# hjxwhy/mipnerf_pl

Measured on NVIDIA H100. Metric: rays/sec (4096-ray batch, 128+128 samples), higher is better.
Workload: dtype bf16

## Files before the change

mipnerf_pl_b200/csrc/mlp_tc.cu:

```cuda
#include "mlp_tc.h"

#include <algorithm>
#include <cstdlib>
#include <mutex>

#include "kernels.h"
#include "profile.h"
#include "ray_math.cuh"
#include "ray_resample.cuh"
#include "tc_common.cuh"

namespace mipnerf {
namespace {

using namespace tc;

constexpr int kN = 128;
constexpr int kWidth = 256;
constexpr int kCond = 128;
constexpr int kFeat = 96;
constexpr int kViewDim = 27;
constexpr int kNumLayers = 10;
constexpr uint32_t kStageBytes = 16384;
constexpr uint32_t kTailBytes = 8192;
// ... 169 lines not shown

template <int kFmt>
__device__ __forceinline__ float2 unpack2(uint32_t v) {
  if (kFmt == 1) return __bfloat1622float2(*reinterpret_cast<__nv_bfloat162*>(&v));
  return __half22float2(*reinterpret_cast<__half2*>(&v));
}
template <int kFmt>
__device__ __forceinline__ void store8_split(uint8_t* dst_hi, uint8_t* dst_lo, const float (&x)[8]) {
  uint32_t h[4], l[4];
#pragma unroll
  for (int e = 0; e < 4; ++e) {
    h[e] = pack2<kFmt>(x[2 * e], x[2 * e + 1]);
    const float2 f = unpack2<kFmt>(h[e]);
    l[e] = pack2<kFmt>(x[2 * e] - f.x, x[2 * e + 1] - f.y);
  }
  *reinterpret_cast<uint4*>(dst_hi) = make_uint4(h[0], h[1], h[2], h[3]);
  *reinterpret_cast<uint4*>(dst_lo) = make_uint4(l[0], l[1], l[2], l[3]);
}

template <int kFmt, bool kX3, int kT, bool kDensity = false>
__device__ __forceinline__ void ipe_row_group(const LevelParams& p, const RayGeom& g, int64_t ray, int row, float t0,
                                              float t1, uint8_t* myF, int gi_begin, int gi_end) {
  float mean[3] = {0.f, 0.f, 0.f}, cov[3] = {0.f, 0.f, 0.f};
  const float* fin = nullptr;
  if (kDensity) {
    const int64_t pt = ray * kN + row;
    if (pt < p.num_points) {
#pragma unroll
      for (int c = 0; c < 3; ++c) {
        mean[c] = __ldg(p.q_means + pt * 3 + c);
        cov[c] = p.q_covs && !p.disable_integration ? __ldg(p.q_covs + pt * 3 + c) : 0.f;
      }
    }
  } else if (kT == 1 && p.feat_in) {
    fin = p.feat_in + (ray * kN + row) * kFeat;
  } else {
    float tm, tv, rv;
    frustum_moments(t0, t1, g.radius_sq, tm, tv, rv);
    lift_gaussian(g, tm, tv, rv, mean, cov);
    if (p.disable_integration) cov[0] = cov[1] = cov[2] = 0.f;
  }
#pragma unroll
  for (int gi = 0; gi < 6; ++gi) {
    if (gi < gi_begin || gi >= gi_end) continue;
    float fsin[8], fcos[8];
    if (fin) {
#pragma unroll
      for (int e = 0; e < 8; ++e) {
        fsin[e] = __ldg(fin + gi * 8 + e);
        fcos[e] = __ldg(fin + 48 + gi * 8 + e);
      }
    } else {
#pragma unroll
      for (int e = 0; e < 8; ++e) {
        const int f = gi * 8 + e;
        ipe_pair<!kDensity>(mean[f % 3], cov[f % 3], f / 3, fsin[e], fcos[e]);
      }
    }
    const uint32_t o_sin = sw128_offset(row, gi * 8);
    const uint32_t o_cos = gi < 2 ? sw128_offset(row, 48 + gi * 8)
                                  : kStageBytes + sw64_offset(row, (gi - 2) * 8);
    if (kX3) {
      store8_split<kFmt>(myF + o_sin, myF + kFBytes + o_sin, fsin);
      store8_split<kFmt>(myF + o_cos, myF + kFBytes + o_cos, fcos);
    } else {
      store8<kFmt>(myF + o_sin, fsin);
      store8<kFmt>(myF + o_cos, fcos);
    }
  }
}

constexpr int kThreads = 384;
constexpr int kHelperWarp0 = 9;
constexpr int kHelperThreads = 96;
constexpr int kHelperBar = 3;
constexpr int kHeadsWriters = 2 * 128 / 4;
#ifndef MIPNERF_LEVEL_PRODUCER_REGS
#define MIPNERF_LEVEL_PRODUCER_REGS 40
#endif
constexpr int kProducerRegs = MIPNERF_LEVEL_PRODUCER_REGS;
constexpr int kConsumerRegs = (65536 / 128 - kProducerRegs) / 2 / 8 * 8;
static_assert(2 * 128 * kConsumerRegs + 128 * kProducerRegs <= 65536 && kProducerRegs % 8 == 0, "setmaxnreg split");
#ifndef MIPNERF_LEVEL_STAGES
#define MIPNERF_LEVEL_STAGES 6
#endif
template <bool kX3, int kT>
struct LevelLayout {
  static constexpr int kFeatBufs = kX3 ? 1 : 2;
  static constexpr uint32_t kFBuf = (kX3 ? 2 : 1) * kFBytes;
  static constexpr int kStages = kX3 ? 2 : MIPNERF_LEVEL_STAGES;
  static constexpr uint32_t kStage = 16384;
  static constexpr uint32_t kA = 0;
  static constexpr uint32_t kF = kA + (kX3 ? 2 * kABytes : 0);
  static constexpr uint32_t kW = kF + kFeatBufs * kFBuf;
  static constexpr uint32_t kMisc = kW + kStages * kStage;
  static constexpr int kNumMbars = 2 * kStages + 2 * kFeatBufs + 2 * 2;
  static constexpr uint32_t kMiscBytes =
      kNumMbars * 8 + 2 * kN * 4 * 4 + 4 * kT * 4 + 4 * kT * 8 * 4 + (kT * kN + 1) * 4;
  static constexpr uint32_t kVBias = (kMisc + kMiscBytes + 15) & ~15u;
  static constexpr uint32_t kVBiasBytes = 2 * kCond * 4;
  static constexpr uint32_t kPhase = kVBias + kVBiasBytes;
  static constexpr uint32_t kTotal = kPhase + kPhaseBytes + 1024;
  static_assert(kT == 1 || kT == 2, "a ray is one or two 128-row tiles");
  static_assert(kNumMbars % 2 == 0, "the raw heads behind the mbarriers must be 16-B aligned");
  static_assert(kTotal <= 232448, "exceeds 227 KB of shared memory per CTA");
  static_assert(kX3 || kStages * kStage > 72 * 1024 || kTotal + 1024 <= 132 * 1024,
                "bf16 / fp16 with a weight ring of up to 72 KB no longer fits the 132 KB carveout");
  static_assert(kX3 || kStages * kStage > 96 * 1024 || kTotal + 1024 <= 164 * 1024,
                "bf16 / fp16 with a weight ring of up to 96 KB no longer fits the 164 KB carveout");
  static_assert(kX3 ? kStage == 2 * w_stage(false, 0, 0).bytes : kStage == w_stage(true, 1, 0).bytes,
                "a ring slot holds one stage (split modes: its hi and lo stages)");
};

__device__ __forceinline__ bool level_reads_feat(int l, int k) { return l == 0 || (l == 5 && k >= kWidth); }
__device__ __forceinline__ uint64_t level_a_desc(int l, int k, uint32_t a_u, uint32_t f_u, uint32_t ft_u) {
  if (!level_reads_feat(l, k)) return make_sw128_desc(a_u + (uint32_t)(k >> 6) * kStageBytes + 2u * (uint32_t)(k & 63));
  const int kf = l == 0 ? k : k - kWidth;
  if (kf < 64) return make_sw128_desc(f_u + 2u * (uint32_t)kf);
  return make_sw64_desc(ft_u + 2u * (uint32_t)(kf - 64));
}

struct RingPos {
  int st;
  uint32_t ph;
  int prev;
};

template <bool kX3>
__device__ __forceinline__ uint32_t level_stage_acquire(uint32_t w_u, uint64_t* w_full, const RingPos& rp,
                                                        PhaseClock& clk) {
  mbar_wait(&w_full[rp.st], rp.ph);
  clk.mark(kPhWFull);
  wgmma_fence();
  return w_u + (uint32_t)rp.st * LevelLayout<kX3, 1>::kStage;
}
template <bool kX3>
__device__ __forceinline__ void level_stage_commit(uint64_t* w_empty, RingPos& rp, bool leader, PhaseClock& clk) {
  wgmma_commit();
  wgmma_wait<1>();
  if (rp.prev >= 0 && leader) mbar_arrive(&w_empty[rp.prev]);
  rp.prev = rp.st;
  if (++rp.st == LevelLayout<kX3, 1>::kStages) {
    rp.st = 0;
    rp.ph ^= 1;
  }
  clk.mark(kPhMma);
}
template <int kFmt, bool kX3>
__device__ __forceinline__ void level_mma_slab(float (&acc)[64], int l, int s, uint32_t a_u, uint32_t f_u,
                                               uint32_t ft_u, uint32_t w_u, uint64_t* w_full, uint64_t* w_empty,
                                               RingPos& rp, bool leader, PhaseClock& clk) {
  const uint32_t b_u = level_stage_acquire<kX3>(w_u, w_full, rp, clk);
  const WStage ws = w_stage(!kX3, l, s);
#pragma unroll
  for (int j = 0; j < 4; ++j) {
    if (16 * j >= ws.kw) break;
    const uint64_t a_hi = level_a_desc(l, ws.k0 + 16 * j, a_u, f_u, ft_u);
    const uint64_t b_hi = ws.sw128 ? make_sw128_desc(b_u + 32u * j) : make_sw64_desc(b_u + 32u * j);
    wgmma_m64n128k16<kFmt>(acc, a_hi, b_hi, (s | j) ? 1u : 0u);
    if (kX3) {
      wgmma_m64n128k16<kFmt>(acc, a_hi + (level_reads_feat(l, ws.k0) ? kFBytes : kABytes) / 16, b_hi, 1u);
      wgmma_m64n128k16<kFmt>(acc, a_hi, b_hi + ws.bytes / 16, 1u);
    }
  }
  level_stage_commit<kX3>(w_empty, rp, leader, clk);
}
template <int kFmt>
__device__ __forceinline__ void level_mma_slab_rs(float (&acc)[64], const uint32_t (&x)[64], int s, uint32_t w_u,
                                                  uint64_t* w_full, uint64_t* w_empty, RingPos& rp, bool leader,
                                                  PhaseClock& clk) {
  const uint32_t b_u = level_stage_acquire<false>(w_u, w_full, rp, clk);
#pragma unroll
  for (int j = 0; j < 4; ++j) {
    const uint32_t a[4] = {x[16 * s + 4 * j], x[16 * s + 4 * j + 1], x[16 * s + 4 * j + 2], x[16 * s + 4 * j + 3]};
    wgmma_m64n128k16_rs<kFmt>(acc, a, make_sw128_desc(b_u + 32u * j), (s | j) ? 1u : 0u);
  }
  level_stage_commit<false>(w_empty, rp, leader, clk);
}

constexpr int kEpiChunks = 4;
constexpr int kEpiGroups = 16 / kEpiChunks;
constexpr int kEpiOverlap = 1;
static_assert(kEpiOverlap >= 1 && kEpiOverlap + kEpiChunks <= 8, "chunk c must follow the retirement of K-slab c");

struct EpiConsts {
  float2 b[kEpiGroups];
};
__device__ __forceinline__ void level_epilogue_consts(EpiConsts& e, int l, int c_base, int chunk, int cq,
                                                      const SmallParams* __restrict__ gsp) {
#pragma unroll
  for (int jj = 0; jj < kEpiGroups; ++jj)
    e.b[jj] = __ldg(reinterpret_cast<const float2*>(gsp->bias[l] + c_base + 8 * (kEpiGroups * chunk + jj) + cq));
}

template <int kFmt, bool kX3>
__device__ __forceinline__ void level_epilogue_chunk(const float (&acc)[64], const EpiConsts& e, int l, int c_base,
                                                     int chunk, int r0, int cq, uint8_t* sA,
                                                     const SmallParams* __restrict__ gsp, float& d0, float& d1) {
  const bool relu = l < 8;
  uint32_t row_off = (uint32_t)r0 * 128u + 2u * (uint32_t)cq, sw = (uint32_t)(r0 & 7) << 4;
  asm volatile("" : "+r"(row_off), "+r"(sw));
#pragma unroll
  for (int jj = 0; jj < kEpiGroups; ++jj) {
    const int j = kEpiGroups * chunk + jj;
    const float2 b = e.b[jj];
    float a0 = acc[4 * j], a1 = acc[4 * j + 1], a2 = acc[4 * j + 2], a3 = acc[4 * j + 3];
    fadd2(a0, a1, b.x, b.y);
    fadd2(a2, a3, b.x, b.y);
    if (l == 7) {
      const float2 wd = __ldg(reinterpret_cast<const float2*>(gsp->w_density + c_base + 8 * j + cq));
      ffma2(d0, d1, fmaxf(a0, 0.f), fmaxf(a2, 0.f), wd.x, wd.x);
      ffma2(d0, d1, fmaxf(a1, 0.f), fmaxf(a3, 0.f), wd.y, wd.y);
    }
    if (relu) a0 = fmaxf(a0, 0.f), a1 = fmaxf(a1, 0.f), a2 = fmaxf(a2, 0.f), a3 = fmaxf(a3, 0.f);
    const uint32_t o0 = (uint32_t)((c_base >> 6) + (j >> 3)) * kStageBytes + (row_off | ((uint32_t)(j & 7) << 4 ^ sw));
    const uint32_t o1 = o0 + 8u * 128u;
    const uint32_t h0 = pack2<kFmt>(a0, a1), h1 = pack2<kFmt>(a2, a3);
    *reinterpret_cast<uint32_t*>(sA + o0) = h0;
    *reinterpret_cast<uint32_t*>(sA + o1) = h1;
    if (kX3) {
      const float2 f0 = unpack2<kFmt>(h0), f1 = unpack2<kFmt>(h1);
      *reinterpret_cast<uint32_t*>(sA + kABytes + o0) = pack2<kFmt>(a0 - f0.x, a1 - f0.y);
      *reinterpret_cast<uint32_t*>(sA + kABytes + o1) = pack2<kFmt>(a2 - f1.x, a3 - f1.y);
    }
  }
}

#ifndef MIPNERF_LEVEL_EPI_FIRST
#define MIPNERF_LEVEL_EPI_FIRST 4
#endif
constexpr int kEpiFirstRs = MIPNERF_LEVEL_EPI_FIRST;
static_assert(kEpiFirstRs >= 0 && kEpiFirstRs + kEpiChunks <= 8, "the chunks must follow K-slabs 0..3");
__host__ __device__ constexpr int epi_slab_acc0(int c) { return (kEpiFirstRs + c) / 2; }
__host__ __device__ constexpr int epi_slab_acc1(int c) { return c / 2; }
static_assert(epi_slab_acc1(kEpiChunks - 1) < 2, "acc1's chunks must land before the next layer's K-slab 2 reads them");

struct LevelRsCtx {
  uint32_t f_u, ft_u, w_u;
  uint64_t* w_full;
  uint64_t* w_empty;
  uint64_t* feat_empty;
  const SmallParams* gsp;
  uint8_t* dump;
  size_t dump_stride;
  uint64_t dump_policy;
  int r0, cq;
  bool leader;
};

template <int kFmt>
__device__ __forceinline__ void level_epilogue_chunk_rs(const float (&acc)[64], const EpiConsts& e, int l, int c_base,
                                                        int chunk, uint32_t (&x)[64], const LevelRsCtx& k, float& d0,
                                                        float& d1) {
  const bool relu = l < 8;
  uint8_t* dump = k.dump ? k.dump + (size_t)l * k.dump_stride : nullptr;
#pragma unroll
  for (int jj = 0; jj < kEpiGroups; ++jj) {
    const int j = kEpiGroups * chunk + jj;
    const float2 b = e.b[jj];
    float a0 = acc[4 * j], a1 = acc[4 * j + 1], a2 = acc[4 * j + 2], a3 = acc[4 * j + 3];
    fadd2(a0, a1, b.x, b.y);
    fadd2(a2, a3, b.x, b.y);
    if (l == 7) {
      const float2 wd = __ldg(reinterpret_cast<const float2*>(k.gsp->w_density + c_base + 8 * j + k.cq));
      ffma2(d0, d1, fmaxf(a0, 0.f), fmaxf(a2, 0.f), wd.x, wd.x);
      ffma2(d0, d1, fmaxf(a1, 0.f), fmaxf(a3, 0.f), wd.y, wd.y);
    }
    if (relu) a0 = fmaxf(a0, 0.f), a1 = fmaxf(a1, 0.f), a2 = fmaxf(a2, 0.f), a3 = fmaxf(a3, 0.f);
    const int jg = (c_base >> 3) + j;
    x[2 * jg] = pack2<kFmt>(a0, a1);
    x[2 * jg + 1] = pack2<kFmt>(a2, a3);
  }
  if (dump) {
    const int q = k.cq >> 1;
    const int jg = (c_base >> 3) + kEpiGroups * chunk + q;
    const uint32_t o0 = (uint32_t)(jg >> 3) * kStageBytes + sw128_offset(k.r0, 8 * (jg & 7));
#pragma unroll
    for (int h = 0; h < 2; ++h) {
      uint32_t v[4];
#pragma unroll
      for (int jj = 0; jj < 4; ++jj) v[jj] = x[2 * ((c_base >> 3) + kEpiGroups * chunk + jj) + h];
#pragma unroll
      for (int i = 0; i < 2; ++i) {
        const uint32_t r = __shfl_xor_sync(0xffffffffu, (q & 2) ? v[i] : v[2 + i], 2);
        if (q & 2) v[i] = r;
        else v[2 + i] = r;
      }
#pragma unroll
      for (int i = 0; i < 2; ++i) {
        const uint32_t r = __shfl_xor_sync(0xffffffffu, (q & 1) ? v[2 * i] : v[2 * i + 1], 1);
        if (q & 1) v[2 * i] = r;
        else v[2 * i + 1] = r;
      }
      st_global_v4_hint(dump + o0 + (uint32_t)h * 8u * 128u, make_uint4(v[0], v[1], v[2], v[3]), k.dump_policy);
    }
  }
}

template <int kFmt>
__device__ __forceinline__ void level_rs_next_head(float (&acc0)[64], float (&acc1)[64], uint32_t (&x)[64], int l,
                                                   bool release_feat, const LevelRsCtx& k, RingPos& rp, PhaseClock& clk,
                                                   float& d0, float& d1) {
  wgmma_fence_acc(acc0);
#pragma unroll
  for (int s = 0; s < 2; ++s) {
    EpiConsts e[kEpiChunks];
#pragma unroll
    for (int c = 0; c < kEpiChunks; ++c)
      if (epi_slab_acc1(c) == s) level_epilogue_consts(e[c], l, 128, c, k.cq, k.gsp);
    level_mma_slab_rs<kFmt>(acc0, x, s, k.w_u, k.w_full, k.w_empty, rp, k.leader, clk);
    if (s == 0 && release_feat && k.leader) mbar_arrive(k.feat_empty);
    if (s == 0) wgmma_fence_acc(acc1);
#pragma unroll
    for (int c = 0; c < kEpiChunks; ++c)
      if (epi_slab_acc1(c) == s) level_epilogue_chunk_rs<kFmt>(acc1, e[c], l, 128, c, x, k, d0, d1);
    clk.mark(kPhEpilogue);
  }
}

template <int kFmt, bool kSkip, bool kLast = false>
__device__ __forceinline__ void level_rs_layer(float (&acc0)[64], float (&acc1)[64], const uint32_t (&x_in)[64],
                                               uint32_t (&x_out)[64], int l, const LevelRsCtx& k, RingPos& rp,
                                               PhaseClock& clk, float& d0, float& d1) {
  const bool skip = kSkip && l == 5;
  uint32_t f_u = k.f_u, ft_u = k.ft_u;
  asm volatile("" : "+r"(f_u), "+r"(ft_u));
#pragma unroll
  for (int s = 2; s < kWidth / 64; ++s)
    level_mma_slab_rs<kFmt>(acc0, x_in, s, k.w_u, k.w_full, k.w_empty, rp, k.leader, clk);
  if (skip) {
#pragma unroll
    for (int s = kWidth / 64; s < num_slabs(true, 5); ++s)
      level_mma_slab<kFmt, false>(acc0, 5, s, 0u, f_u, ft_u, k.w_u, k.w_full, k.w_empty, rp, k.leader, clk);
  }
  wgmma_fence_acc(acc1);
#pragma unroll
  for (int s = 0; s < kWidth / 64; ++s) {
    EpiConsts e[kEpiChunks];
#pragma unroll
    for (int c = 0; c < kEpiChunks; ++c)
      if (epi_slab_acc0(c) == s) level_epilogue_consts(e[c], l, 0, c, k.cq, k.gsp);
    level_mma_slab_rs<kFmt>(acc1, x_in, s, k.w_u, k.w_full, k.w_empty, rp, k.leader, clk);
    if (s == epi_slab_acc0(0)) wgmma_fence_acc(acc0);
#pragma unroll
    for (int c = 0; c < kEpiChunks; ++c)
      if (epi_slab_acc0(c) == s) level_epilogue_chunk_rs<kFmt>(acc0, e[c], l, 0, c, x_out, k, d0, d1);
    clk.mark(kPhEpilogue);
  }
  if (skip) {
#pragma unroll
    for (int s = kWidth / 64; s < num_slabs(true, 5); ++s)
      level_mma_slab<kFmt, false>(acc1, 5, s, 0u, f_u, ft_u, k.w_u, k.w_full, k.w_empty, rp, k.leader, clk);
  }
  if constexpr (kLast) {
    wgmma_wait<0>();
    wgmma_fence_acc(acc1);
    if (k.leader) mbar_arrive(&k.w_empty[rp.prev]);
    rp.prev = -1;
    clk.mark(kPhMma);
#pragma unroll
    for (int c = 0; c < kEpiChunks; ++c) {
      EpiConsts e;
      level_epilogue_consts(e, l, 128, c, k.cq, k.gsp);
      level_epilogue_chunk_rs<kFmt>(acc1, e, l, 128, c, x_out, k, d0, d1);
    }
    clk.mark(kPhEpilogue);
  } else {
    level_rs_next_head<kFmt>(acc0, acc1, x_out, l, skip, k, rp, clk, d0, d1);
  }
}

__device__ __forceinline__ float quad_sum(float v) {
  v += __shfl_xor_sync(0xffffffffu, v, 1);
  return v + __shfl_xor_sync(0xffffffffu, v, 2);
}

constexpr int kViewPts = 4;
__device__ __forceinline__ float view_enc_elem(const float* vd, int f, int num_deg) {
  float enc;
  if (f < 3) {
    enc = __ldg(vd + f);
  } else {
    const int gidx = f - 3, half = 3 * num_deg, is_cos = gidx >= half, h = is_cos ? gidx - half : gidx;
    const float y = __fmul_rn(__ldg(vd + h % 3), __int_as_float((127 + h / 3) << 23));
    enc = sinf(is_cos ? __fadd_rn(y, MIPNERF_HALF_PI_F32) : y);
  }
  return enc;
}
__device__ __forceinline__ void level_view_terms(const LevelParams& p, int64_t tile, float* slot, int hw, int lane) {
  const float4* wt = reinterpret_cast<const float4*>(p.wimage + kViewDirOffset);
  const float4 b4 = __ldg(wt + kViewDim * kCond / 4 + lane);
#pragma unroll 1
  for (int r = kViewPts * hw; r < kN; r += kViewPts * (kHelperThreads / 32)) {
    float enc[kViewPts];
#pragma unroll
    for (int q = 0; q < kViewPts; ++q) {
      const int64_t pt = tile * kN + r + q;
      enc[q] = 0.f;
      if (lane < kViewDim && pt < p.num_points) {
        const float* vd = p.viewdirs + pt * 3;
        if (lane < 3) {
          enc[q] = __ldg(vd + lane);
        } else {
          const int gidx = lane - 3, is_cos = gidx >= 12, h = is_cos ? gidx - 12 : gidx;
          const float y = __fmul_rn(__ldg(vd + h % 3), __int_as_float((127 + h / 3) << 23));
          enc[q] = sinf(is_cos ? __fadd_rn(y, MIPNERF_HALF_PI_F32) : y);
        }
      }
    }
    float acc[kViewPts][4];
#pragma unroll
    for (int q = 0; q < kViewPts; ++q) acc[q][0] = b4.x, acc[q][1] = b4.y, acc[q][2] = b4.z, acc[q][3] = b4.w;
#pragma unroll 3
    for (int k = 0; k < kViewDim; ++k) {
      const float4 w4 = __ldg(wt + k * (kCond / 4) + lane);
#pragma unroll
      for (int q = 0; q < kViewPts; ++q) {
        const float e = __shfl_sync(0xffffffffu, enc[q], k);
        acc[q][0] = fmaf(w4.x, e, acc[q][0]);
        acc[q][1] = fmaf(w4.y, e, acc[q][1]);
        acc[q][2] = fmaf(w4.z, e, acc[q][2]);
        acc[q][3] = fmaf(w4.w, e, acc[q][3]);
      }
    }
#pragma unroll
    for (int q = 0; q < kViewPts; ++q)
      __stcg(reinterpret_cast<float4*>(slot + (r + q) * kCond) + lane,
             make_float4(acc[q][0], acc[q][1], acc[q][2], acc[q][3]));
  }
  __threadfence_block();
}

template <int kFmt, bool kX3, int kT, int kMode = kModeForward>
__device__ __forceinline__ void level_prepare_tile(const LevelParams& p, int64_t ray, int tt, uint8_t* fbuf,
                                                   float* rs_scratch, int ht, int hw, int lane, PhaseClock& clk,
                                                   float* vb_slot, float* vslot = nullptr) {
  constexpr int kNs = kT * kN;
  constexpr bool kDensity = kMode != kModeForward;
  if constexpr (kMode == kModeRadiance) {
    level_view_terms(p, ray, vslot, hw, lane);
    clk.mark(kPhPrologue);
  }
  if (!kDensity && (kT == 1 || tt == 0)) {
    if (hw == 0) {
      float* t_ray = p.t + ray * (kNs + 1);
      if (p.t_mode == 1) {
        const float nr = __ldg(p.near + ray), fr = __ldg(p.far + ray);
        const bool jit = draws_active(p.t_rand);
// ... 254 lines not shown
            mbar_wait(&feat_empty[fb], ((uint32_t)(j / Lay::kFeatBufs) & 1u) ^ 1u);
            clk.mark(kPhFeatEmpty);
            level_prepare_tile<kFmt, kX3, kT, kMode>(
                p, ray, tt, sF + fb * Lay::kFBuf, rs_scratch, ht, hw, lane, clk, vbias + (i & 1) * kCond,
                kMode == kModeRadiance ? p.view_bias + ((size_t)blockIdx.x * 2 + (j & 1)) * (kN * kCond) : nullptr);
            mbar_arrive(&feat_full[fb]);
          }
          if (tt == 0 && i > 0) {
            const int par = (int)(((i - 1) * kT) & 1);
#pragma unroll
            for (int u = 0; u < kT; ++u)
              mbar_wait(&heads_full[par + u], (uint32_t)(((i - 1) * kT + u) >> 1) & 1u);
            clk.mark(kPhHeadsFull);
            if constexpr (kDensity || kMode == kModeViewAcc)
              level_density_out(p, ray - gridDim.x, heads + par * kN * 4, &heads_empty[par], ht, clk);
            else if constexpr (kMode == kModeRadiance)
              level_radiance_out(p, ray - gridDim.x, heads + par * kN * 4, &heads_empty[par], ht, clk);
            else
              level_composite_ray<kT>(p, ray - gridDim.x, heads + par * kN * 4, &heads_empty[par], cs, ps, ht, hw, lane,
                                      clk);
          }
        }
        if (!more) break;
      }
      clk.end(phase_slot, 3);
      return;
    }
    if (lane == 0) {
      clk.begin(phase_rows + 2 * kNumPhases, true);
      int st = 0;
      uint32_t ph = 0;
      const uint64_t pol = l2_policy_evict_last();
      for (int64_t tile = 0, ray = blockIdx.x; ray < p.num_rays; ray += ++tile % kT == 0 ? gridDim.x : 0) {
        const uint8_t* src = p.wimage;
        for (int l = 0; l < (kDensity ? 8 : kNumLayers); ++l)
          for (int h = 0; h < num_halves(l); ++h)
            for (int s = 0; s < num_slabs(!kX3, l); ++s) {
              const uint32_t bytes = w_stage(!kX3, l, s).bytes;
              clk.mark(kPhIssue);
              mbar_wait(&w_empty[st], ph ^ 1);
              clk.mark(kPhWEmpty);
              mbar_arrive_expect_tx(&w_full[st], kX3 ? 2 * bytes : bytes);
              bulk_g2s_hint(sW + st * Lay::kStage, src, bytes, &w_full[st], pol);
              if (kX3) bulk_g2s_hint(sW + st * Lay::kStage + bytes, src + kLoOffset, bytes, &w_full[st], pol);
              src += bytes;
              if (++st == Lay::kStages) {
                st = 0;
                ph ^= 1;
              }
            }
      }
      clk.mark(kPhIssue);
      clk.end(phase_slot, 2);
    }
    return;
  }

  asm volatile("setmaxnreg.inc.sync.aligned.u32 %0;\n" ::"n"(kConsumerRegs) : "memory");
  const int wg = warp >> 2, t = tid & 127, wq = warp & 3;
  const int r0 = 64 * wg + 16 * wq + (lane >> 2);
  const int cq = 2 * (lane & 3);
  const bool leader = t == 0;
  const SmallParams* __restrict__ gsp = reinterpret_cast<const SmallParams*>(p.wimage + kSmallOffset);
  const uint32_t a_u = smem_u32(sA) + (uint32_t)wg * 64u * 128u;
  const uint32_t w_u = smem_u32(sW);
  const uint64_t dump_policy =
      (kMode != kModeRadiance || kQueryDump) && kT == 1 && p.act_dump ? l2_policy_evict_first() : 0ull;
  bool dump_pending = false;
  RingPos rp{0, 0u, -1};
  clk.begin(phase_rows + wg * kNumPhases, leader);
  for (int64_t ray = blockIdx.x, i = 0; ray < p.num_rays; ray += ++i % kT == 0 ? gridDim.x : 0) {
    const int fb = (int)(i % Lay::kFeatBufs), par = (int)(i & 1);
    const uint32_t fph = (uint32_t)(i / Lay::kFeatBufs) & 1u, hph = (uint32_t)(i >> 1) & 1u;
    const int vpar = kT == 1 ? par : (int)hph;
    const uint32_t f_u = smem_u32(sF) + (uint32_t)fb * Lay::kFBuf + (uint32_t)wg * 64u * 128u;
    const uint32_t ft_u = smem_u32(sF) + (uint32_t)fb * Lay::kFBuf + kStageBytes + (uint32_t)wg * 64u * 64u;
    mbar_wait(&feat_full[fb], fph);
    clk.mark(kPhFeatFull);

    float d0 = 0.f, d1 = 0.f;
    float rgb[2][3] = {{0.f, 0.f, 0.f}, {0.f, 0.f, 0.f}};
    float acc0[64], acc1[64];
    wgmma_fence_acc(acc0);
#pragma unroll
    for (int s = 0; s < num_slabs(!kX3, 0); ++s)
      level_mma_slab<kFmt, kX3>(acc0, 0, s, a_u, f_u, ft_u, w_u, w_full, w_empty, rp, leader, clk);
    if constexpr (!kX3) {
      const LevelRsCtx k{f_u, ft_u, w_u, w_full, w_empty, &feat_empty[fb], gsp,
                         kDumps && kT == 1 && p.act_dump ? p.act_dump + (size_t)ray * kABytes : nullptr,
                         (size_t)p.dump_tiles * kABytes, dump_policy, r0, cq, leader};
      uint32_t xa[64], xb[64];
      static_assert(2 * num_slabs(true, 0) == kEpiChunks, "layer 0: two acc0 chunks after each of its K-slabs");
      wgmma_fence_acc(acc1);
#pragma unroll
      for (int s = 0; s < num_slabs(true, 0); ++s) {
        EpiConsts e[2];
        level_epilogue_consts(e[0], 0, 0, 2 * s, cq, gsp);
        level_epilogue_consts(e[1], 0, 0, 2 * s + 1, cq, gsp);
        level_mma_slab<kFmt, false>(acc1, 0, s, a_u, f_u, ft_u, w_u, w_full, w_empty, rp, leader, clk);
        if (s == 0) wgmma_fence_acc(acc0);
        level_epilogue_chunk_rs<kFmt>(acc0, e[0], 0, 0, 2 * s, xb, k, d0, d1);
        level_epilogue_chunk_rs<kFmt>(acc0, e[1], 0, 0, 2 * s + 1, xb, k, d0, d1);
        clk.mark(kPhEpilogue);
      }
      level_rs_next_head<kFmt>(acc0, acc1, xb, 0, false, k, rp, clk, d0, d1);
#pragma unroll 1
      for (int l = 1; l < (kDensity ? 7 : 9); l += 2) {
        level_rs_layer<kFmt, true>(acc0, acc1, xb, xa, l, k, rp, clk, d0, d1);
        level_rs_layer<kFmt, false>(acc0, acc1, xa, xb, l + 1, k, rp, clk, d0, d1);
      }
      if constexpr (kDensity) {
        level_rs_layer<kFmt, false, true>(acc0, acc1, xb, xa, 7, k, rp, clk, d0, d1);
      } else {
#pragma unroll
        for (int s = 2; s < num_slabs(true, 9); ++s)
          level_mma_slab_rs<kFmt>(acc0, xb, s, w_u, w_full, w_empty, rp, leader, clk);
      }
    } else {
      for (int l = 0; l < 9; ++l) {
        if (l > 0)
          for (int s = kEpiChunks; s < num_slabs(false, l); ++s)
            level_mma_slab<kFmt, kX3>(acc0, l, s, a_u, f_u, ft_u, w_u, w_full, w_empty, rp, leader, clk);
        wgmma_fence_acc(acc1);
        const int first = l == 0 ? 0 : kEpiOverlap;
        for (int s = 0; s < first; ++s)
          level_mma_slab<kFmt, kX3>(acc1, l, s, a_u, f_u, ft_u, w_u, w_full, w_empty, rp, leader, clk);
#pragma unroll
        for (int c = 0; c < kEpiChunks; ++c) {
          EpiConsts e;
          level_epilogue_consts(e, l, 0, c, cq, gsp);
          if (first + c < num_slabs(false, l))
            level_mma_slab<kFmt, kX3>(acc1, l, first + c, a_u, f_u, ft_u, w_u, w_full, w_empty, rp, leader, clk);
          if (c == 0) {
            wgmma_fence_acc(acc0);
            if (dump_pending) {
              if (leader) bulk_store_wait_read();
              dump_pending = false;
              clk.mark(kPhEpilogue);
              named_bar_sync(1 + wg, 128);
              clk.mark(kPhBarrier);
            }
          }
          level_epilogue_chunk<kFmt, kX3>(acc0, e, l, 0, c, r0, cq, sA, gsp, d0, d1);
          clk.mark(kPhEpilogue);
        }
        for (int s = first + kEpiChunks; s < num_slabs(false, l); ++s)
          level_mma_slab<kFmt, kX3>(acc1, l, s, a_u, f_u, ft_u, w_u, w_full, w_empty, rp, leader, clk);
        if (kDensity && l == 7) break;
        fence_proxy_async_smem();
        clk.mark(kPhEpilogue);
        named_bar_sync(1 + wg, 128);
        clk.mark(kPhBarrier);
        wgmma_fence_acc(acc0);
#pragma unroll
        for (int c = 0; c < kEpiChunks; ++c) {
          EpiConsts e;
          level_epilogue_consts(e, l, 128, c, cq, gsp);
          if (c < kEpiChunks - 1) {
            level_mma_slab<kFmt, kX3>(acc0, l + 1, c, a_u, f_u, ft_u, w_u, w_full, w_empty, rp, leader, clk);
            if (c == 0 && l == 5 && leader) mbar_arrive(&feat_empty[fb]);
            if (c == 0) wgmma_fence_acc(acc1);
          }
          level_epilogue_chunk<kFmt, kX3>(acc1, e, l, 128, c, r0, cq, sA, gsp, d0, d1);
          clk.mark(kPhEpilogue);
        }
        level_mma_slab<kFmt, kX3>(acc0, l + 1, kEpiChunks - 1, a_u, f_u, ft_u, w_u, w_full, w_empty, rp, leader, clk);
        fence_proxy_async_smem();
        clk.mark(kPhEpilogue);
        named_bar_sync(1 + wg, 128);
        clk.mark(kPhBarrier);
        if (kMode != kModeRadiance && kT == 1 && p.act_dump) {
          if (leader) {
#pragma unroll
            for (int k = 0; k < 4; ++k) {
              const uint32_t o = (uint32_t)k * kStageBytes + (uint32_t)wg * 8192u;
              bulk_s2g_hint(p.act_dump + ((size_t)l * p.dump_tiles + ray) * kABytes + o, sA + o, 8192u, dump_policy);
              if constexpr (kTrain)
                bulk_s2g_hint(p.act_dump + ((size_t)(9 + l) * p.dump_tiles + ray) * kABytes + o, sA + kABytes + o, 8192u,
                              dump_policy);
            }
          }
          dump_pending = true;
          clk.mark(kPhEpilogue);
        }
      }
      if constexpr (kDensity) {
        wgmma_wait<0>();
        wgmma_fence_acc(acc1);
        if (leader) mbar_arrive(&w_empty[rp.prev]);
        rp.prev = -1;
        clk.mark(kPhMma);
#pragma unroll
        for (int c = 0; c < kEpiChunks; ++c) {
          EpiConsts e;
          level_epilogue_consts(e, 7, 128, c, cq, gsp);
          level_epilogue_chunk<kFmt, kX3>(acc1, e, 7, 128, c, r0, cq, sA, gsp, d0, d1);
        }
        clk.mark(kPhEpilogue);
      } else {
        for (int s = kEpiChunks; s < num_slabs(false, 9); ++s)
          level_mma_slab<kFmt, kX3>(acc0, 9, s, a_u, f_u, ft_u, w_u, w_full, w_empty, rp, leader, clk);
      }
    }
    if constexpr (kMode == kModeViewAcc) {
      wgmma_wait<0>();
      wgmma_fence_acc(acc0);
      if (leader) mbar_arrive(&w_empty[rp.prev]);
      rp.prev = -1;
      clk.mark(kPhMma);
      const uint64_t pol = l2_policy_evict_first();
      float* va = p.view_acc + ((size_t)ray * kN + r0) * kCond + cq;
#pragma unroll
      for (int j = 0; j < 16; ++j) {
        st_global_v2_hint(va + 8 * j, acc0[4 * j], acc0[4 * j + 1], pol);
        st_global_v2_hint(va + 8 * kCond + 8 * j, acc0[4 * j + 2], acc0[4 * j + 3], pol);
      }
    } else if constexpr (!kDensity) {
      const float* vs = vbias + vpar * kCond + cq;
      float2 vbr[16];
      if constexpr (kMode == kModeForward && !kX3) {
#pragma unroll
        for (int j = 0; j < 16; ++j) vbr[j] = *reinterpret_cast<const float2*>(vs + 8 * j);
      }
      wgmma_wait<0>();
      wgmma_fence_acc(acc0);
      if (leader) mbar_arrive(&w_empty[rp.prev]);
      rp.prev = -1;
      clk.mark(kPhMma);
      const float* vb = p.view_bias + ((size_t)blockIdx.x * 2 + par) * (kN * kCond) + (size_t)r0 * kCond;
      uint8_t* vd = kDumps && kT == 1 && p.v_dump ? p.v_dump + (size_t)ray * (2 * kStageBytes) : nullptr;
#pragma unroll
      for (int j = 0; j < 16; ++j) {
        const int c = 8 * j + cq;
        const float2 b = kMode == kModeRadiance ? __ldcg(reinterpret_cast<const float2*>(vb + c))
                         : kX3                  ? *reinterpret_cast<const float2*>(vs + 8 * j)
                                                : vbr[j];
        const float2 b1 = kMode == kModeRadiance ? __ldcg(reinterpret_cast<const float2*>(vb + 8 * kCond + c)) : b;
        float y[4] = {acc0[4 * j], acc0[4 * j + 1], acc0[4 * j + 2], acc0[4 * j + 3]};
        fadd2(y[0], y[1], b.x, b.y);
        fadd2(y[2], y[3], b1.x, b1.y);
#pragma unroll
        for (int e = 0; e < 4; ++e) y[e] = fmaxf(y[e], 0.f);
#pragma unroll
        for (int ch = 0; ch < 3; ++ch) {
          const float2 wc = __ldg(reinterpret_cast<const float2*>(gsp->w_color[ch] + c));
          ffma2(rgb[0][ch], rgb[1][ch], y[0], y[2], wc.x, wc.x);
          ffma2(rgb[0][ch], rgb[1][ch], y[1], y[3], wc.y, wc.y);
        }
        if (vd) {
          *reinterpret_cast<uint32_t*>(vd + (c >> 6) * kStageBytes + sw128_offset(r0, c & 63)) = pack2<kFmt>(y[0], y[1]);
          *reinterpret_cast<uint32_t*>(vd + (c >> 6) * kStageBytes + sw128_offset(r0 + 8, c & 63)) =
              pack2<kFmt>(y[2], y[3]);
          if constexpr (kTrain) {
            uint8_t* vl = vd + (size_t)p.dump_tiles * (2 * kStageBytes);
            *reinterpret_cast<uint32_t*>(vl + (c >> 6) * kStageBytes + sw128_offset(r0, c & 63)) =
                pack2_low<kFmt>(y[0], y[1], pack2<kFmt>(y[0], y[1]));
            *reinterpret_cast<uint32_t*>(vl + (c >> 6) * kStageBytes + sw128_offset(r0 + 8, c & 63)) =
                pack2_low<kFmt>(y[2], y[3], pack2<kFmt>(y[2], y[3]));
          }
        }
      }
    }
    d0 = quad_sum(d0), d1 = quad_sum(d1);
#pragma unroll
    for (int ch = 0; ch < 3; ++ch) rgb[0][ch] = quad_sum(rgb[0][ch]), rgb[1][ch] = quad_sum(rgb[1][ch]);
    if ((lane & 3) == 0) {
      float* hd = heads + par * kN * 4;
      clk.mark(kPhEpilogue);
      mbar_wait(&heads_empty[par], hph ^ 1);
      clk.mark(kPhBarrier);
      *reinterpret_cast<float4*>(hd + r0 * 4) = make_float4(d0, rgb[0][0], rgb[0][1], rgb[0][2]);
      *reinterpret_cast<float4*>(hd + (r0 + 8) * 4) = make_float4(d1, rgb[1][0], rgb[1][1], rgb[1][2]);
      mbar_arrive(&heads_full[par]);
    }
    clk.mark(kPhEpilogue);
  }
  if (dump_pending && leader) bulk_store_wait_all();
  clk.mark(kPhEpilogue);
  clk.end(phase_slot, wg);
}

__global__ void view_bias_from_enc_kernel(const float* __restrict__ venc, const float* __restrict__ w,
                                          const float* __restrict__ b, float* __restrict__ out, int64_t num_rays) {
  const int64_t idx = (int64_t)blockIdx.x * blockDim.x + threadIdx.x;
  if (idx >= num_rays * kCond) return;
  const int64_t ray = idx / kCond;
  const int n = (int)(idx % kCond);
  float acc = __ldg(b + n);
#pragma unroll
  for (int k = 0; k < kViewDim; ++k)
    acc = fmaf(__ldg(w + (size_t)n * (kWidth + kViewDim) + kWidth + k), __ldg(venc + ray * kViewDim + k), acc);
  out[idx] = acc;
}

__global__ void __launch_bounds__(kCond) view_terms_kernel(const float* __restrict__ dirs, const float* __restrict__ w,
                                                           int64_t sk, int64_t sn, const float* __restrict__ bias,
                                                           int nk, int num_deg, float* __restrict__ terms) {
  __shared__ float enc[kViewDim];
  const int64_t d = blockIdx.x;
  const int n = threadIdx.x;
  if (n < nk) enc[n] = view_enc_elem(dirs + d * 3, n, num_deg);
  __syncthreads();
  float acc = __ldg(bias + n);
  for (int k = 0; k < nk; ++k) acc = fmaf(__ldg(w + k * sk + n * sn), enc[k], acc);
  terms[d * kCond + n] = acc;
}

constexpr int kPairThreads = 128;
constexpr int kPairDirs = 32;
constexpr int kMaxBasis = 16;
// ... 621 lines not shown
```

Measured before the change: 1.848 million.

## Group weight-ring stages in pairs per wgmma commit and deepen ring to eight stages

```diff
diff --git a/mipnerf_pl_b200/csrc/mlp_tc.cu b/mipnerf_pl_b200/csrc/mlp_tc.cu
--- a/mipnerf_pl_b200/csrc/mlp_tc.cu
+++ b/mipnerf_pl_b200/csrc/mlp_tc.cu
@@ -275,13 +275,14 @@
 constexpr int kConsumerRegs = (65536 / 128 - kProducerRegs) / 2 / 8 * 8;
 static_assert(2 * 128 * kConsumerRegs + 128 * kProducerRegs <= 65536 && kProducerRegs % 8 == 0, "setmaxnreg split");
 #ifndef MIPNERF_LEVEL_STAGES
-#define MIPNERF_LEVEL_STAGES 6
+#define MIPNERF_LEVEL_STAGES 8
 #endif
 template <bool kX3, int kT>
 struct LevelLayout {
   static constexpr int kFeatBufs = kX3 ? 1 : 2;
   static constexpr uint32_t kFBuf = (kX3 ? 2 : 1) * kFBytes;
   static constexpr int kStages = kX3 ? 2 : MIPNERF_LEVEL_STAGES;
+  static constexpr int kGroupStages = kX3 ? 1 : 2;
   static constexpr uint32_t kStage = 16384;
   static constexpr uint32_t kA = 0;
   static constexpr uint32_t kF = kA + (kX3 ? 2 * kABytes : 0);
@@ -297,12 +298,16 @@
   static_assert(kT == 1 || kT == 2, "a ray is one or two 128-row tiles");
   static_assert(kNumMbars % 2 == 0, "the raw heads behind the mbarriers must be 16-B aligned");
   static_assert(kTotal <= 232448, "exceeds 227 KB of shared memory per CTA");
-  static_assert(kX3 || kStages * kStage > 72 * 1024 || kTotal + 1024 <= 132 * 1024,
-                "bf16 / fp16 with a weight ring of up to 72 KB no longer fits the 132 KB carveout");
   static_assert(kX3 || kStages * kStage > 96 * 1024 || kTotal + 1024 <= 164 * 1024,
                 "bf16 / fp16 with a weight ring of up to 96 KB no longer fits the 164 KB carveout");
+  static_assert(kX3 || kStages * kStage > 128 * 1024 || kTotal + 1024 <= 196 * 1024,
+                "bf16 / fp16 with a weight ring of up to 128 KB no longer fits the 196 KB carveout");
   static_assert(kX3 ? kStage == 2 * w_stage(false, 0, 0).bytes : kStage == w_stage(true, 1, 0).bytes,
                 "a ring slot holds one stage (split modes: its hi and lo stages)");
+  static_assert(kX3 || (num_slabs(true, 0) % 2 == 0 && num_slabs(true, 1) % 2 == 0 && num_slabs(true, 5) % 2 == 0 &&
+                        num_slabs(true, 9) % 2 == 0),
+                "bf16 / fp16: every layer's K-slabs pair up into groups");
+  static_assert(kStages % kGroupStages == 0, "a commit group's stages must not wrap around the ring");
 };
 
 __device__ __forceinline__ bool level_reads_feat(int l, int k) { return l == 0 || (l == 5 && k >= kWidth); }
@@ -320,55 +325,53 @@
 };
 
 template <bool kX3>
-__device__ __forceinline__ uint32_t level_stage_acquire(uint32_t w_u, uint64_t* w_full, const RingPos& rp,
-                                                        PhaseClock& clk) {
-  mbar_wait(&w_full[rp.st], rp.ph);
-  clk.mark(kPhWFull);
+__device__ __forceinline__ void level_group_acquire(uint32_t (&b_u)[LevelLayout<kX3, 1>::kGroupStages], uint32_t w_u,
+                                                    uint64_t* w_full, const RingPos& rp, PhaseClock& clk) {
+#pragma unroll
+  for (int i = 0; i < LevelLayout<kX3, 1>::kGroupStages; ++i) {
+    mbar_wait(&w_full[rp.st + i], rp.ph);
+    clk.mark(kPhWFull);
+    b_u[i] = w_u + (uint32_t)(rp.st + i) * LevelLayout<kX3, 1>::kStage;
+  }
   wgmma_fence();
-  return w_u + (uint32_t)rp.st * LevelLayout<kX3, 1>::kStage;
 }
 template <bool kX3>
-__device__ __forceinline__ void level_stage_commit(uint64_t* w_empty, RingPos& rp, bool leader, PhaseClock& clk) {
+__device__ __forceinline__ void level_group_release(uint64_t* w_empty, RingPos& rp, bool leader) {
+  if (rp.prev >= 0 && leader) {
+#pragma unroll
+    for (int i = 0; i < LevelLayout<kX3, 1>::kGroupStages; ++i) mbar_arrive(&w_empty[rp.prev + i]);
+  }
+  rp.prev = -1;
+}
+template <bool kX3>
+__device__ __forceinline__ void level_group_commit(uint64_t* w_empty, RingPos& rp, bool leader, PhaseClock& clk) {
   wgmma_commit();
   wgmma_wait<1>();
-  if (rp.prev >= 0 && leader) mbar_arrive(&w_empty[rp.prev]);
+  level_group_release<kX3>(w_empty, rp, leader);
   rp.prev = rp.st;
-  if (++rp.st == LevelLayout<kX3, 1>::kStages) {
+  rp.st += LevelLayout<kX3, 1>::kGroupStages;
+  if (rp.st == LevelLayout<kX3, 1>::kStages) {
     rp.st = 0;
     rp.ph ^= 1;
   }
   clk.mark(kPhMma);
 }
-template <int kFmt, bool kX3>
-__device__ __forceinline__ void level_mma_slab(float (&acc)[64], int l, int s, uint32_t a_u, uint32_t f_u,
-                                               uint32_t ft_u, uint32_t w_u, uint64_t* w_full, uint64_t* w_empty,
-                                               RingPos& rp, bool leader, PhaseClock& clk) {
-  const uint32_t b_u = level_stage_acquire<kX3>(w_u, w_full, rp, clk);
-  const WStage ws = w_stage(!kX3, l, s);
-#pragma unroll
-  for (int j = 0; j < 4; ++j) {
-    if (16 * j >= ws.kw) break;
+template <int kFmt>
+__device__ __forceinline__ void level_mma_slab_x3(float (&acc)[64], int l, int s, uint32_t a_u, uint32_t f_u,
+                                                  uint32_t ft_u, uint32_t w_u, uint64_t* w_full, uint64_t* w_empty,
+                                                  RingPos& rp, bool leader, PhaseClock& clk) {
+  uint32_t b_u[1];
+  level_group_acquire<true>(b_u, w_u, w_full, rp, clk);
+  const WStage ws = w_stage(false, l, s);
+#pragma unroll
+  for (int j = 0; j < 2; ++j) {
     const uint64_t a_hi = level_a_desc(l, ws.k0 + 16 * j, a_u, f_u, ft_u);
-    const uint64_t b_hi = ws.sw128 ? make_sw128_desc(b_u + 32u * j) : make_sw64_desc(b_u + 32u * j);
+    const uint64_t b_hi = make_sw64_desc(b_u[0] + 32u * j);
     wgmma_m64n128k16<kFmt>(acc, a_hi, b_hi, (s | j) ? 1u : 0u);
-    if (kX3) {
-      wgmma_m64n128k16<kFmt>(acc, a_hi + (level_reads_feat(l, ws.k0) ? kFBytes : kABytes) / 16, b_hi, 1u);
-      wgmma_m64n128k16<kFmt>(acc, a_hi, b_hi + ws.bytes / 16, 1u);
-    }
-  }
-  level_stage_commit<kX3>(w_empty, rp, leader, clk);
-}
-template <int kFmt>
-__device__ __forceinline__ void level_mma_slab_rs(float (&acc)[64], const uint32_t (&x)[64], int s, uint32_t w_u,
-                                                  uint64_t* w_full, uint64_t* w_empty, RingPos& rp, bool leader,
-                                                  PhaseClock& clk) {
-  const uint32_t b_u = level_stage_acquire<false>(w_u, w_full, rp, clk);
-#pragma unroll
-  for (int j = 0; j < 4; ++j) {
-    const uint32_t a[4] = {x[16 * s + 4 * j], x[16 * s + 4 * j + 1], x[16 * s + 4 * j + 2], x[16 * s + 4 * j + 3]};
-    wgmma_m64n128k16_rs<kFmt>(acc, a, make_sw128_desc(b_u + 32u * j), (s | j) ? 1u : 0u);
-  }
-  level_stage_commit<false>(w_empty, rp, leader, clk);
+    wgmma_m64n128k16<kFmt>(acc, a_hi + (level_reads_feat(l, ws.k0) ? kFBytes : kABytes) / 16, b_hi, 1u);
+    wgmma_m64n128k16<kFmt>(acc, a_hi, b_hi + ws.bytes / 16, 1u);
+  }
+  level_group_commit<true>(w_empty, rp, leader, clk);
 }
 
 constexpr int kEpiChunks = 4;
@@ -419,14 +422,6 @@
   }
 }
 
-#ifndef MIPNERF_LEVEL_EPI_FIRST
-#define MIPNERF_LEVEL_EPI_FIRST 4
-#endif
-constexpr int kEpiFirstRs = MIPNERF_LEVEL_EPI_FIRST;
-static_assert(kEpiFirstRs >= 0 && kEpiFirstRs + kEpiChunks <= 8, "the chunks must follow K-slabs 0..3");
-__host__ __device__ constexpr int epi_slab_acc0(int c) { return (kEpiFirstRs + c) / 2; }
-__host__ __device__ constexpr int epi_slab_acc1(int c) { return c / 2; }
-static_assert(epi_slab_acc1(kEpiChunks - 1) < 2, "acc1's chunks must land before the next layer's K-slab 2 reads them");
 
 struct LevelRsCtx {
   uint32_t f_u, ft_u, w_u;
@@ -490,25 +485,50 @@
   }
 }
 
+template <int kFmt, bool kFeat>
+__device__ __forceinline__ void level_mma_group(float (&acc)[64], const uint32_t (&x)[64], int l, int g, uint32_t f_u,
+                                                uint32_t ft_u, const LevelRsCtx& k, RingPos& rp, PhaseClock& clk) {
+  uint32_t b_u[2];
+  level_group_acquire<false>(b_u, k.w_u, k.w_full, rp, clk);
+#pragma unroll
+  for (int i = 0; i < 2; ++i) {
+    const int s = 2 * g + i;
+    const WStage ws = w_stage(true, kFeat ? l : 1, s);
+#pragma unroll
+    for (int j = 0; j < 4; ++j) {
+      if (16 * j >= ws.kw) break;
+      const uint64_t b = ws.sw128 ? make_sw128_desc(b_u[i] + 32u * j) : make_sw64_desc(b_u[i] + 32u * j);
+      if constexpr (kFeat) {
+        wgmma_m64n128k16<kFmt>(acc, level_a_desc(l, ws.k0 + 16 * j, 0u, f_u, ft_u), b, (s | j) ? 1u : 0u);
+      } else {
+        const uint32_t a[4] = {x[16 * s + 4 * j], x[16 * s + 4 * j + 1], x[16 * s + 4 * j + 2], x[16 * s + 4 * j + 3]};
+        wgmma_m64n128k16_rs<kFmt>(acc, a, b, (s | j) ? 1u : 0u);
+      }
+    }
+  }
+  level_group_commit<false>(k.w_empty, rp, k.leader, clk);
+}
+
+template <int kFmt>
+__device__ __forceinline__ void level_epilogue_rs(const float (&acc)[64], int l, int c_base, uint32_t (&x)[64],
+                                                  const LevelRsCtx& k, float& d0, float& d1) {
+  EpiConsts e[kEpiChunks];
+#pragma unroll
+  for (int c = 0; c < kEpiChunks; ++c) level_epilogue_consts(e[c], l, c_base, c, k.cq, k.gsp);
+#pragma unroll
+  for (int c = 0; c < kEpiChunks; ++c) level_epilogue_chunk_rs<kFmt>(acc, e[c], l, c_base, c, x, k, d0, d1);
+}
+
 template <int kFmt>
 __device__ __forceinline__ void level_rs_next_head(float (&acc0)[64], float (&acc1)[64], uint32_t (&x)[64], int l,
                                                    bool release_feat, const LevelRsCtx& k, RingPos& rp, PhaseClock& clk,
                                                    float& d0, float& d1) {
   wgmma_fence_acc(acc0);
-#pragma unroll
-  for (int s = 0; s < 2; ++s) {
-    EpiConsts e[kEpiChunks];
-#pragma unroll
-    for (int c = 0; c < kEpiChunks; ++c)
-      if (epi_slab_acc1(c) == s) level_epilogue_consts(e[c], l, 128, c, k.cq, k.gsp);
-    level_mma_slab_rs<kFmt>(acc0, x, s, k.w_u, k.w_full, k.w_empty, rp, k.leader, clk);
-    if (s == 0 && release_feat && k.leader) mbar_arrive(k.feat_empty);
-    if (s == 0) wgmma_fence_acc(acc1);
-#pragma unroll
-    for (int c = 0; c < kEpiChunks; ++c)
-      if (epi_slab_acc1(c) == s) level_epilogue_chunk_rs<kFmt>(acc1, e[c], l, 128, c, x, k, d0, d1);
-    clk.mark(kPhEpilogue);
-  }
+  level_mma_group<kFmt, false>(acc0, x, l + 1, 0, 0u, 0u, k, rp, clk);
+  if (release_feat && k.leader) mbar_arrive(k.feat_empty);
+  wgmma_fence_acc(acc1);
+  level_epilogue_rs<kFmt>(acc1, l, 128, x, k, d0, d1);
+  clk.mark(kPhEpilogue);
 }
 
 template <int kFmt, bool kSkip, bool kLast = false>
@@ -518,45 +538,21 @@
   const bool skip = kSkip && l == 5;
   uint32_t f_u = k.f_u, ft_u = k.ft_u;
   asm volatile("" : "+r"(f_u), "+r"(ft_u));
-#pragma unroll
-  for (int s = 2; s < kWidth / 64; ++s)
-    level_mma_slab_rs<kFmt>(acc0, x_in, s, k.w_u, k.w_full, k.w_empty, rp, k.leader, clk);
-  if (skip) {
-#pragma unroll
-    for (int s = kWidth / 64; s < num_slabs(true, 5); ++s)
-      level_mma_slab<kFmt, false>(acc0, 5, s, 0u, f_u, ft_u, k.w_u, k.w_full, k.w_empty, rp, k.leader, clk);
-  }
+  level_mma_group<kFmt, false>(acc0, x_in, l, 1, 0u, 0u, k, rp, clk);
+  if (skip) level_mma_group<kFmt, true>(acc0, x_in, 5, 2, f_u, ft_u, k, rp, clk);
   wgmma_fence_acc(acc1);
-#pragma unroll
-  for (int s = 0; s < kWidth / 64; ++s) {
-    EpiConsts e[kEpiChunks];
-#pragma unroll
-    for (int c = 0; c < kEpiChunks; ++c)
-      if (epi_slab_acc0(c) == s) level_epilogue_consts(e[c], l, 0, c, k.cq, k.gsp);
-    level_mma_slab_rs<kFmt>(acc1, x_in, s, k.w_u, k.w_full, k.w_empty, rp, k.leader, clk);
-    if (s == epi_slab_acc0(0)) wgmma_fence_acc(acc0);
-#pragma unroll
-    for (int c = 0; c < kEpiChunks; ++c)
-      if (epi_slab_acc0(c) == s) level_epilogue_chunk_rs<kFmt>(acc0, e[c], l, 0, c, x_out, k, d0, d1);
-    clk.mark(kPhEpilogue);
-  }
-  if (skip) {
-#pragma unroll
-    for (int s = kWidth / 64; s < num_slabs(true, 5); ++s)
-      level_mma_slab<kFmt, false>(acc1, 5, s, 0u, f_u, ft_u, k.w_u, k.w_full, k.w_empty, rp, k.leader, clk);
-  }
+  level_mma_group<kFmt, false>(acc1, x_in, l, 0, 0u, 0u, k, rp, clk);
+  level_mma_group<kFmt, false>(acc1, x_in, l, 1, 0u, 0u, k, rp, clk);
+  wgmma_fence_acc(acc0);
+  level_epilogue_rs<kFmt>(acc0, l, 0, x_out, k, d0, d1);
+  clk.mark(kPhEpilogue);
+  if (skip) level_mma_group<kFmt, true>(acc1, x_in, 5, 2, f_u, ft_u, k, rp, clk);
   if constexpr (kLast) {
     wgmma_wait<0>();
     wgmma_fence_acc(acc1);
-    if (k.leader) mbar_arrive(&k.w_empty[rp.prev]);
-    rp.prev = -1;
+    level_group_release<false>(k.w_empty, rp, k.leader);
     clk.mark(kPhMma);
-#pragma unroll
-    for (int c = 0; c < kEpiChunks; ++c) {
-      EpiConsts e;
-      level_epilogue_consts(e, l, 128, c, k.cq, k.gsp);
-      level_epilogue_chunk_rs<kFmt>(acc1, e, l, 128, c, x_out, k, d0, d1);
-    }
+    level_epilogue_rs<kFmt>(acc1, l, 128, x_out, k, d0, d1);
     clk.mark(kPhEpilogue);
   } else {
     level_rs_next_head<kFmt>(acc0, acc1, x_out, l, skip, k, rp, clk, d0, d1);
@@ -977,27 +973,18 @@
     float rgb[2][3] = {{0.f, 0.f, 0.f}, {0.f, 0.f, 0.f}};
     float acc0[64], acc1[64];
     wgmma_fence_acc(acc0);
-#pragma unroll
-    for (int s = 0; s < num_slabs(!kX3, 0); ++s)
-      level_mma_slab<kFmt, kX3>(acc0, 0, s, a_u, f_u, ft_u, w_u, w_full, w_empty, rp, leader, clk);
     if constexpr (!kX3) {
       const LevelRsCtx k{f_u, ft_u, w_u, w_full, w_empty, &feat_empty[fb], gsp,
                          kDumps && kT == 1 && p.act_dump ? p.act_dump + (size_t)ray * kABytes : nullptr,
                          (size_t)p.dump_tiles * kABytes, dump_policy, r0, cq, leader};
       uint32_t xa[64], xb[64];
-      static_assert(2 * num_slabs(true, 0) == kEpiChunks, "layer 0: two acc0 chunks after each of its K-slabs");
+      static_assert(num_slabs(true, 0) == 2, "layer 0: one group per N-half");
+      level_mma_group<kFmt, true>(acc0, xa, 0, 0, f_u, ft_u, k, rp, clk);
       wgmma_fence_acc(acc1);
-#pragma unroll
-      for (int s = 0; s < num_slabs(true, 0); ++s) {
-        EpiConsts e[2];
-        level_epilogue_consts(e[0], 0, 0, 2 * s, cq, gsp);
-        level_epilogue_consts(e[1], 0, 0, 2 * s + 1, cq, gsp);
-        level_mma_slab<kFmt, false>(acc1, 0, s, a_u, f_u, ft_u, w_u, w_full, w_empty, rp, leader, clk);
-        if (s == 0) wgmma_fence_acc(acc0);
-        level_epilogue_chunk_rs<kFmt>(acc0, e[0], 0, 0, 2 * s, xb, k, d0, d1);
-        level_epilogue_chunk_rs<kFmt>(acc0, e[1], 0, 0, 2 * s + 1, xb, k, d0, d1);
-        clk.mark(kPhEpilogue);
-      }
+      level_mma_group<kFmt, true>(acc1, xa, 0, 0, f_u, ft_u, k, rp, clk);
+      wgmma_fence_acc(acc0);
+      level_epilogue_rs<kFmt>(acc0, 0, 0, xb, k, d0, d1);
+      clk.mark(kPhEpilogue);
       level_rs_next_head<kFmt>(acc0, acc1, xb, 0, false, k, rp, clk, d0, d1);
 #pragma unroll 1
       for (int l = 1; l < (kDensity ? 7 : 9); l += 2) {
@@ -1007,25 +994,26 @@
       if constexpr (kDensity) {
         level_rs_layer<kFmt, false, true>(acc0, acc1, xb, xa, 7, k, rp, clk, d0, d1);
       } else {
-#pragma unroll
-        for (int s = 2; s < num_slabs(true, 9); ++s)
-          level_mma_slab_rs<kFmt>(acc0, xb, s, w_u, w_full, w_empty, rp, leader, clk);
+        level_mma_group<kFmt, false>(acc0, xb, 9, 1, 0u, 0u, k, rp, clk);
       }
     } else {
+#pragma unroll
+      for (int s = 0; s < num_slabs(false, 0); ++s)
+        level_mma_slab_x3<kFmt>(acc0, 0, s, a_u, f_u, ft_u, w_u, w_full, w_empty, rp, leader, clk);
       for (int l = 0; l < 9; ++l) {
         if (l > 0)
           for (int s = kEpiChunks; s < num_slabs(false, l); ++s)
-            level_mma_slab<kFmt, kX3>(acc0, l, s, a_u, f_u, ft_u, w_u, w_full, w_empty, rp, leader, clk);
+            level_mma_slab_x3<kFmt>(acc0, l, s, a_u, f_u, ft_u, w_u, w_full, w_empty, rp, leader, clk);
         wgmma_fence_acc(acc1);
         const int first = l == 0 ? 0 : kEpiOverlap;
         for (int s = 0; s < first; ++s)
-          level_mma_slab<kFmt, kX3>(acc1, l, s, a_u, f_u, ft_u, w_u, w_full, w_empty, rp, leader, clk);
+          level_mma_slab_x3<kFmt>(acc1, l, s, a_u, f_u, ft_u, w_u, w_full, w_empty, rp, leader, clk);
 #pragma unroll
         for (int c = 0; c < kEpiChunks; ++c) {
           EpiConsts e;
           level_epilogue_consts(e, l, 0, c, cq, gsp);
           if (first + c < num_slabs(false, l))
-            level_mma_slab<kFmt, kX3>(acc1, l, first + c, a_u, f_u, ft_u, w_u, w_full, w_empty, rp, leader, clk);
+            level_mma_slab_x3<kFmt>(acc1, l, first + c, a_u, f_u, ft_u, w_u, w_full, w_empty, rp, leader, clk);
           if (c == 0) {
             wgmma_fence_acc(acc0);
             if (dump_pending) {
@@ -1040,7 +1028,7 @@
           clk.mark(kPhEpilogue);
         }
         for (int s = first + kEpiChunks; s < num_slabs(false, l); ++s)
-          level_mma_slab<kFmt, kX3>(acc1, l, s, a_u, f_u, ft_u, w_u, w_full, w_empty, rp, leader, clk);
+          level_mma_slab_x3<kFmt>(acc1, l, s, a_u, f_u, ft_u, w_u, w_full, w_empty, rp, leader, clk);
         if (kDensity && l == 7) break;
         fence_proxy_async_smem();
         clk.mark(kPhEpilogue);
@@ -1052,14 +1040,14 @@
           EpiConsts e;
           level_epilogue_consts(e, l, 128, c, cq, gsp);
           if (c < kEpiChunks - 1) {
-            level_mma_slab<kFmt, kX3>(acc0, l + 1, c, a_u, f_u, ft_u, w_u, w_full, w_empty, rp, leader, clk);
+            level_mma_slab_x3<kFmt>(acc0, l + 1, c, a_u, f_u, ft_u, w_u, w_full, w_empty, rp, leader, clk);
             if (c == 0 && l == 5 && leader) mbar_arrive(&feat_empty[fb]);
             if (c == 0) wgmma_fence_acc(acc1);
           }
           level_epilogue_chunk<kFmt, kX3>(acc1, e, l, 128, c, r0, cq, sA, gsp, d0, d1);
           clk.mark(kPhEpilogue);
         }
-        level_mma_slab<kFmt, kX3>(acc0, l + 1, kEpiChunks - 1, a_u, f_u, ft_u, w_u, w_full, w_empty, rp, leader, clk);
+        level_mma_slab_x3<kFmt>(acc0, l + 1, kEpiChunks - 1, a_u, f_u, ft_u, w_u, w_full, w_empty, rp, leader, clk);
         fence_proxy_async_smem();
         clk.mark(kPhEpilogue);
         named_bar_sync(1 + wg, 128);
@@ -1082,8 +1070,7 @@
       if constexpr (kDensity) {
         wgmma_wait<0>();
         wgmma_fence_acc(acc1);
-        if (leader) mbar_arrive(&w_empty[rp.prev]);
-        rp.prev = -1;
+        level_group_release<kX3>(w_empty, rp, leader);
         clk.mark(kPhMma);
 #pragma unroll
         for (int c = 0; c < kEpiChunks; ++c) {
@@ -1094,14 +1081,13 @@
         clk.mark(kPhEpilogue);
       } else {
         for (int s = kEpiChunks; s < num_slabs(false, 9); ++s)
-          level_mma_slab<kFmt, kX3>(acc0, 9, s, a_u, f_u, ft_u, w_u, w_full, w_empty, rp, leader, clk);
+          level_mma_slab_x3<kFmt>(acc0, 9, s, a_u, f_u, ft_u, w_u, w_full, w_empty, rp, leader, clk);
       }
     }
     if constexpr (kMode == kModeViewAcc) {
       wgmma_wait<0>();
       wgmma_fence_acc(acc0);
-      if (leader) mbar_arrive(&w_empty[rp.prev]);
-      rp.prev = -1;
+      level_group_release<kX3>(w_empty, rp, leader);
       clk.mark(kPhMma);
       const uint64_t pol = l2_policy_evict_first();
       float* va = p.view_acc + ((size_t)ray * kN + r0) * kCond + cq;
@@ -1119,8 +1105,7 @@
       }
       wgmma_wait<0>();
       wgmma_fence_acc(acc0);
-      if (leader) mbar_arrive(&w_empty[rp.prev]);
-      rp.prev = -1;
+      level_group_release<kX3>(w_empty, rp, leader);
       clk.mark(kPhMma);
       const float* vb = p.view_bias + ((size_t)blockIdx.x * 2 + par) * (kN * kCond) + (size_t)r0 * kCond;
       uint8_t* vd = kDumps && kT == 1 && p.v_dump ? p.v_dump + (size_t)ray * (2 * kStageBytes) : nullptr;
```

Measured after the change: 1.894 million, median of 6. 2.5% higher.
